# ISU-PAAL/DeepDFA

Measured on NVIDIA H100. Metric: CFG graphs/sec (train step), higher is better.
Workload: dtype f32 (GRU GEMMs: bf16x3 split operands, f32 accumulate)

## Files before the change

deepdfa_b200/csrc/gru_tc_bwd.cu:

```cuda
#include <cuda_fp16.h>

#include <atomic>

#include "tc_common.cuh"

namespace ddfa {
namespace tc2b {
using namespace tcc;

constexpr int kThreads = 320, kEpiWarps = 8;

constexpr int kGbWarps = 8;
struct GbRow {
  float4 d, hv, rr, zz, nn, gh;
  float deg;
  int tb, te;
};
__device__ __forceinline__ float4 bf16x4_to_f4(const uint2 &p) {
  return make_float4(__uint_as_float(p.x << 16), __uint_as_float(p.x & 0xffff0000u), __uint_as_float(p.y << 16), __uint_as_float(p.y & 0xffff0000u));
}
__device__ __forceinline__ void gb_load(GbRow &x, const float *__restrict__ dh_out, const float *__restrict__ h,
                                        const uint8_t *__restrict__ h_img_src, const float *__restrict__ gates,
                                        const uint4 *__restrict__ gates_packed, const int32_t *__restrict__ indptr,
                                        const int32_t *__restrict__ indptr_t, size_t plane, int64_t node, int col, bool ok,
// ... 346 lines not shown
    mbar_init(w_full, 1);
    mbar_fence_init();
  }
  __syncthreads();
  if (threadIdx.x == 0) trace_stamp(tron, 0, 0);
  pdl_launch_dependents();

  if (warp == kEpiWarps) {
    const uint64_t pol_saved = l2_policy((hints & 2) ? 1 : 0), pol_dh = l2_policy((hints & 8) ? 1 : 0);
    const uint64_t pol_q = l2_policy((hints & 64) ? 1 : 0);
    if (my_tiles > 0 && elect_one()) {
      mbar_arrive_expect_tx(w_full, kD3WBytes);
      bulk_g2s(sbase, packed3 + (size_t)rh * kD3WBytes, kD3WBytes, w_full);
    }
    __syncwarp();
    pdl_wait();
    int cc = 0;
    for (int k = 0; k < my_tiles; ++k, cc += 4) {
      const int tile = tile_of(k);
      if (elect_one()) {
        const int stage = cc % kD3Stages, use = cc / kD3Stages;
        if (use > 0) mbar_wait_bounded(empty(stage), (use - 1) & 1);
        const int64_t r0 = (int64_t)tile * kTileM + kGtRows * rh;
        const int valid = (int)max((int64_t)0, min((int64_t)kGtRows, (int64_t)N - r0));
        const uint32_t dst = sbase + kD3OffStage + stage * kD3StageBytes;
        const uint32_t bytes = (uint32_t)valid * (kD * 4 + kD * 8) + (HF32 ? (uint32_t)valid * kD * 4 : (uint32_t)kGtRows * kD * 4);
        mbar_arrive_expect_tx(full(stage), bytes);
        if (valid > 0) {
          bulk_g2s_hint(dst + kGtOffD, dh_out + r0 * kD, (uint32_t)valid * kD * 4, full(stage), pol_dh);
          bulk_g2s_hint(dst + kGtOffG, gates_packed + r0 * kD, (uint32_t)valid * kD * 8, full(stage), pol_saved);
        }
        if (HF32) {
          if (valid > 0) bulk_g2s_hint(dst + kGtOffH, h + r0 * kD, (uint32_t)valid * kD * 4, full(stage), pol_saved);
        } else {
          const uint8_t *t0 = h_img_src + (size_t)tile * kImageTileBytes + (size_t)(kGtRows * rh) * 128;
#pragma unroll
          for (int ch = 0; ch < 4; ++ch) bulk_g2s_hint(dst + kGtOffH + ch * (kGtRows * 128), t0 + (size_t)ch * kChunkBytes, kGtRows * 128, full(stage), pol_saved);
        }
      }
      __syncwarp();
      cluster_arrive_release();
      cluster_wait_acquire();
      if (elect_one()) {
        fence_proxy_async_global();
        for (int g = 0; g < 3; ++g) {
          const int m = g < 2 ? g : (role == 0 ? 2 : 3);
          const int c = cc + 1 + g, stage = c % kD3Stages, use = c / kD3Stages;
          if (use > 0) mbar_wait_bounded(empty(stage), (use - 1) & 1);
          mbar_arrive_expect_tx(full(stage), kD3StageBytes);
          bulk_g2s_hint(sbase + kD3OffStage + stage * kD3StageBytes, q_img + (size_t)m * img_stride + (size_t)tile * kImageTileBytes,
                        kD3StageBytes, full(stage), pol_q);
          if (g != 1) trace_stamp(tron, k, g == 0 ? 1 : 2);
        }
      }
      __syncwarp();
    }
  } else {
    pdl_wait();
    const int col = lane * 4;
#define DDFA_POL_TMP l2_policy((hints & 4) ? 2 : 0)
    const int wg = warp >> 2;
    const bool tr = (warp == 0 && lane == 0);
    float4 sum[7];
#pragma unroll
    for (int i = 0; i < 7; ++i) sum[i] = make_float4(0.f, 0.f, 0.f, 0.f);
    static_assert(kGtPre == 2 && kGtRowsPerWarp == 4, "lane slots below assume four rows per warp and two prefetched neighbours per row");
    auto node_of = [&](int tile, int r) { return (int64_t)tile * kTileM + kGtRows * rh + warp + kEpiWarps * r; };
    auto load_scalars = [&](int kk) -> int {
      int v = 0;
      if (kk < my_tiles && lane < 16) {
        const int64_t nd = node_of(tile_of(kk), (lane >> 1) & 3);
        const int32_t *base = lane < 8 ? indptr : indptr_t;
        if (nd < N && base) v = __ldcg(base + nd + (lane & 1));
      }
      return v;
    };
    auto load_ids = [&](int sc) -> int {
      const int r_ = (lane >> 1) & 3, q_ = lane & 1;
      const int tb_ = __shfl_sync(0xffffffffu, sc, 8 + 2 * r_), te_ = __shfl_sync(0xffffffffu, sc, 9 + 2 * r_);
      int v = -1;
      if (lane >= 16 && lane < 24 && tb_ + q_ < te_) v = __ldcg(indices_t + tb_ + q_);
      return v;
    };
    int sc_cur = 0, sc_next = 0, id_cur = -1;
    if constexpr (CSRP) {
      sc_cur = load_scalars(0); sc_next = load_scalars(1);
      id_cur = load_ids(sc_cur);
    }
    int cc = 0;
    for (int k = 0; k < my_tiles; ++k) {
      const int tile = tile_of(k);
      {
        const int stage = cc % kD3Stages, use = cc / kD3Stages;
        ++cc;
        const int64_t node0 = node_of(tile, 0);
        bool ok[kGtRowsPerWarp];
        int tb[kGtRowsPerWarp], te[kGtRowsPerWarp];
        float deg[kGtRowsPerWarp];
        int id[kGtRowsPerWarp][kGtPre];
        if constexpr (CSRP) {
          const int sc_next2 = load_scalars(k + 2);
          const int id_next = load_ids(sc_next);
#pragma unroll
          for (int r = 0; r < kGtRowsPerWarp; ++r) {
            ok[r] = node0 + kEpiWarps * r < N;
            deg[r] = (float)(__shfl_sync(0xffffffffu, sc_cur, 2 * r + 1) - __shfl_sync(0xffffffffu, sc_cur, 2 * r));
            tb[r] = __shfl_sync(0xffffffffu, sc_cur, 8 + 2 * r); te[r] = __shfl_sync(0xffffffffu, sc_cur, 9 + 2 * r);
#pragma unroll
            for (int q = 0; q < kGtPre; ++q) id[r][q] = __shfl_sync(0xffffffffu, id_cur, 16 + 2 * r + q);
          }
          sc_cur = sc_next; sc_next = sc_next2; id_cur = id_next;
        } else {
#pragma unroll
          for (int r = 0; r < kGtRowsPerWarp; ++r) {
            const int64_t nd = node0 + kEpiWarps * r;
            ok[r] = nd < N;
            tb[r] = te[r] = 0;
            deg[r] = 0.f;
            if (ok[r]) {
              deg[r] = (float)(__ldcg(indptr + nd + 1) - __ldcg(indptr + nd));
              if (indptr_t) { tb[r] = __ldcg(indptr_t + nd); te[r] = __ldcg(indptr_t + nd + 1); }
            }
          }
#pragma unroll
          for (int r = 0; r < kGtRowsPerWarp; ++r)
#pragma unroll
            for (int q = 0; q < kGtPre; ++q) id[r][q] = (tb[r] + q < te[r]) ? __ldcg(indices_t + tb[r] + q) : -1;
        }
        float4 gv[kGtRowsPerWarp][kGtPre];
#pragma unroll
        for (int r = 0; r < kGtRowsPerWarp; ++r)
#pragma unroll
          for (int q = 0; q < kGtPre; ++q) gv[r][q] = id[r][q] >= 0 ? ldg_cg_f4(ds_in + (size_t)id[r][q] * kD + col) : make_float4(0.f, 0.f, 0.f, 0.f);
        mbar_wait_bounded(full(stage), use & 1);
        const uint8_t *st = smem + kD3OffStage + stage * kD3StageBytes;
#pragma unroll
        for (int r = 0; r < kGtRowsPerWarp; ++r) {
          const int row = warp + kEpiWarps * r;
          float4 d = make_float4(0.f, 0.f, 0.f, 0.f), hv = d, rr = d, zz = d, nn = d, gh = d;
          if (ok[r]) {
            d = *reinterpret_cast<const float4 *>(st + kGtOffD + row * (kD * 4) + col * 4);
            const uint4 g0 = *reinterpret_cast<const uint4 *>(st + kGtOffG + row * (kD * 8) + col * 8);
            const uint4 g1 = *reinterpret_cast<const uint4 *>(st + kGtOffG + row * (kD * 8) + col * 8 + 16);
            unpack_gates(make_uint2(g0.x, g0.y), rr.x, zz.x, nn.x, gh.x);
            unpack_gates(make_uint2(g0.z, g0.w), rr.y, zz.y, nn.y, gh.y);
            unpack_gates(make_uint2(g1.x, g1.y), rr.z, zz.z, nn.z, gh.z);
            unpack_gates(make_uint2(g1.z, g1.w), rr.w, zz.w, nn.w, gh.w);
            if (HF32) {
              hv = *reinterpret_cast<const float4 *>(st + kGtOffH + row * (kD * 4) + col * 4);
            } else {
              const uint32_t off = (uint32_t)((col >> 6) * (kGtRows * 128) + row * 128 + (((((col & 63) >> 3) ^ (row & 7)) & 7) << 4) + (col & 7) * 2);
              const uint2 hh = *reinterpret_cast<const uint2 *>(st + kGtOffH + off);
              const uint2 hl = *reinterpret_cast<const uint2 *>(st + kGtOffH + 2 * (kGtRows * 128) + off);
              const float4 a = bf16x4_to_f4(hh), b = bf16x4_to_f4(hl);
              hv = make_float4(a.x + b.x, a.y + b.y, a.z + b.z, a.w + b.w);
            }
#pragma unroll
            for (int q = 0; q < kGtPre; ++q) f4_add(d, gv[r][q]);
            for (int j = tb[r] + kGtPre; j < te[r]; ++j) f4_add(d, ldg_cg_f4(ds_in + (size_t)__ldcg(indices_t + j) * kD + col));
          }
          float4 qr = make_float4(0.f, 0.f, 0.f, 0.f), qz = qr, qn = qr, qnr = qr;
          const int64_t node = node0 + kEpiWarps * r;
          if (ok[r]) {
            st_f4_hint(dh + (size_t)node * kD + col, make_float4(d.x * zz.x, d.y * zz.y, d.z * zz.z, d.w * zz.w), DDFA_POL_TMP);
#define BWDQ2(f)                                         \
  {                                                      \
    const float dz_ = d.f * (hv.f - nn.f);               \
    const float dn_ = d.f * (1.f - zz.f);                \
    qn.f = dn_ * (1.f - nn.f * nn.f);                    \
    qz.f = dz_ * zz.f * (1.f - zz.f);                    \
    qr.f = qn.f * gh.f * rr.f * (1.f - rr.f);            \
    qnr.f = qn.f * rr.f;                                 \
  }
            BWDQ2(x) BWDQ2(y) BWDQ2(z) BWDQ2(w)
#undef BWDQ2
            f4_add(sum[0], qr); f4_add(sum[1], qz); f4_add(sum[2], qn); f4_add(sum[3], qnr);
            f4_fma(sum[4], deg[r], qr); f4_fma(sum[5], deg[r], qz); f4_fma(sum[6], deg[r], qn);
          }
          const size_t o_hi = image_offset(node, col, 0), o_lo = image_offset(node, col, 1);
          uint2 ph, pl;
          split4(qr, ph, pl);  *reinterpret_cast<uint2 *>(q_img + 0 * img_stride + o_hi) = ph; *reinterpret_cast<uint2 *>(q_img + 0 * img_stride + o_lo) = pl;
          split4(qz, ph, pl);  *reinterpret_cast<uint2 *>(q_img + 1 * img_stride + o_hi) = ph; *reinterpret_cast<uint2 *>(q_img + 1 * img_stride + o_lo) = pl;
          split4(qn, ph, pl);  *reinterpret_cast<uint2 *>(q_img + 2 * img_stride + o_hi) = ph; *reinterpret_cast<uint2 *>(q_img + 2 * img_stride + o_lo) = pl;
          split4(qnr, ph, pl); *reinterpret_cast<uint2 *>(q_img + 3 * img_stride + o_hi) = ph; *reinterpret_cast<uint2 *>(q_img + 3 * img_stride + o_lo) = pl;
        }
        __syncwarp();
        if (lane == 0) mbar_arrive(empty(stage));
      }
      if (k > 0 && (warp & 3) == 0) {
        bulk_wait_read_all();
        __syncwarp();
        if (lane == 0) mbar_arrive_n(empty(kD3OutStage), kEpiWarps / 2);
      }
      fence_proxy_async_global();
      cluster_arrive_release();
      cluster_wait_acquire();
      if (tr) trace_stamp(tron, k, 11);
      if ((warp & 3) == 0 && role == 1) fence_proxy_async_global();
      if (k == 0) mbar_wait_bounded(w_full, 0);
      float acc[32];
      int pending = -1;
      if (tr) { trace_stamp(tron, k, 7); trace_stamp(tron, k, 3); }
      for (int g = 0; g < 3; ++g, ++cc) {
        const int stage = cc % kD3Stages, use = cc / kD3Stages;
        mbar_wait_bounded(full(stage), use & 1);
        if (tr && g != 1) trace_stamp(tron, k, g == 0 ? 4 : 5);
        wgmma_fence();
        const uint32_t a0 = sbase + kD3OffStage + stage * kD3StageBytes + wg * 8192;
        const uint32_t w0 = sbase + g * 4 * kD3WChunkBytes;
#pragma unroll
        for (int kb = 0; kb < 2; ++kb) {
#pragma unroll
          for (int k4 = 0; k4 < 4; ++k4) {
            const uint64_t a_hi = gmma_desc(a0 + kb * kChunkBytes + k4 * 32), a_lo = gmma_desc(a0 + (2 + kb) * kChunkBytes + k4 * 32);
            const uint64_t b_hi = gmma_desc(w0 + kb * kD3WChunkBytes + k4 * 32), b_lo = gmma_desc(w0 + (2 + kb) * kD3WChunkBytes + k4 * 32);
            wgmma_n64<0, 0>(acc, a_hi, b_hi, (g == 0 && kb == 0 && k4 == 0) ? 0u : 1u);
            wgmma_n64<0, 0>(acc, a_hi, b_lo, 1u);
            wgmma_n64<0, 0>(acc, a_lo, b_hi, 1u);
          }
        }
        wgmma_commit();
        wgmma_wait<1>();
        __syncwarp();
        if (pending >= 0 && lane == 0) mbar_arrive(empty(pending));
        pending = stage;
      }
      wgmma_wait<0>();
      wgmma_fence_regs(acc);
      if (tr) { trace_stamp(tron, k, 6); trace_stamp(tron, k, 8); trace_stamp(tron, k, 9); }
      const uint32_t st_base = sbase + kD3OffStage + kD3OutStage * kD3StageBytes;
      if (wg == 0) asm volatile("bar.sync 2, 128;" ::: "memory");
      else asm volatile("bar.sync 3, 128;" ::: "memory");
      uint32_t tid;
      asm volatile("mov.u32 %0, %%tid.x;" : "=r"(tid));
#pragma unroll
      for (int hh = 0; hh < 2; ++hh) {
        const uint32_t rowp = staged_row(st_base, wg, (tid >> 5 & 3) * 16 + (tid >> 2 & 7) + 8 * hh) + 8 * (tid & 3);
#pragma unroll
        for (int j = 0; j < 8; ++j)
          asm volatile("st.shared.v2.f32 [%0], {%1, %2};" ::"r"(rowp + 32 * j), "f"(acc[4 * j + 2 * hh]), "f"(acc[4 * j + 2 * hh + 1]) : "memory");
      }
      fence_proxy_async_shared();
      if (wg == 0) asm volatile("bar.sync 2, 128;" ::: "memory");
      else asm volatile("bar.sync 3, 128;" ::: "memory");
      if ((warp & 3) == 0 && elect_one()) {
        const uint64_t pol_tmp = DDFA_POL_TMP;
        const int64_t node0 = (int64_t)tile * kTileM + wg * 64;
        float *out = (role == 0 ? ds : dh) + node0 * kD + half * 64;
        const int rows = (int)min((int64_t)64, (int64_t)N - node0);
        for (int r = 0; r < rows; ++r) {
          if (role == 0) bulk_s2g_hint(out + (int64_t)r * kD, staged_row(st_base, wg, r), 64 * 4, pol_tmp);
          else bulk_s2g_add_f32_hint(out + (int64_t)r * kD, staged_row(st_base, wg, r), 64 * 4, pol_tmp);
        }
        bulk_commit();
      }
      __syncwarp();
      if (tr) trace_stamp(tron, k, 10);
    }
#undef DDFA_POL_TMP
    bulk_wait_all();
    asm volatile("bar.sync 1, %0;" ::"n"(32 * kEpiWarps) : "memory");
    float *red = reinterpret_cast<float *>(smem + kD3OffStage);
#pragma unroll
    for (int i = 0; i < 7; ++i) *reinterpret_cast<float4 *>(&red[(warp * 7 + i) * kD + col]) = sum[i];
  }
  __syncthreads();
  const float *red = reinterpret_cast<const float *>(smem + kD3OffStage);
  for (int i = threadIdx.x; i < 7 * kD; i += kD3Threads) {
    float v_ = 0.f;
#pragma unroll
    for (int w = 0; w < kEpiWarps; ++w) v_ += red[(w * 7) * kD + i];
    if (bias_slots) { bias_slots[(size_t)blockIdx.x * 7 * kD + i] = v_; continue; }
    const int which = i >> 7, c_ = i & 127;
    if (which == 0) { atomicAdd(db_ih + c_, v_); atomicAdd(db_hh + c_, v_); }
    else if (which == 1) { atomicAdd(db_ih + kD + c_, v_); atomicAdd(db_hh + kD + c_, v_); }
    else if (which == 2) atomicAdd(db_ih + 2 * kD + c_, v_);
    else if (which == 3) atomicAdd(db_hh + 2 * kD + c_, v_);
    else atomicAdd(db_fold + (which - 4) * kD + c_, v_);
  }
}

constexpr int kWgSlotBytes = kImageTileBytes;
constexpr int kWgSlots = 3;
constexpr int kWgOffBar = kWgSlots * kWgSlotBytes;
constexpr int kWgSmemAlloc = kWgOffBar + 2 * kWgSlots * 8 + 1024;
constexpr int kWgThreads = 32 * kEpiWarps + 32;
constexpr size_t kWgPartialFloats = (size_t)3 * kD * kD;
constexpr int kWgMaxSteps = 16;
struct WgBatch {
  const uint8_t *s_img[kWgMaxSteps];
  const uint8_t *h_img[kWgMaxSteps];
  int32_t steps;
};
__global__ void __launch_bounds__(kWgThreads, 1) wgrad_kernel(const uint8_t *__restrict__ q_img, size_t img_stride, size_t step_stride,
                                                              const __grid_constant__ WgBatch batch,
                                                              int32_t N, float *__restrict__ partial, int first, int hints) {
  extern __shared__ uint8_t smem_raw[];
  uint8_t *smem = reinterpret_cast<uint8_t *>((reinterpret_cast<uintptr_t>(smem_raw) + 1023) & ~(uintptr_t)1023);
  const uint32_t sbase = smem_u32(smem);
  const uint32_t bar0 = sbase + kWgOffBar;
  auto full = [&](int i) { return bar0 + 8u * i; };
  auto empty = [&](int i) { return bar0 + 8u * (kWgSlots + i); };

  const int warp = threadIdx.x >> 5, lane = threadIdx.x & 31;
  const int role = blockIdx.y / 3, g = blockIdx.y % 3;
  const int qm = g < 2 ? g : (role == 0 ? 2 : 3);
  const int num_tiles = (N + kTileM - 1) / kTileM;
  const int all_tiles = num_tiles * batch.steps;
  const int my_tiles = (all_tiles > (int)blockIdx.x) ? (all_tiles - 1 - (int)blockIdx.x) / (int)gridDim.x + 1 : 0;

  if (threadIdx.x == 0) {
    for (int i = 0; i < kWgSlots; ++i) { mbar_init(full(i), 1); mbar_init(empty(i), kEpiWarps); }
    mbar_fence_init();
  }
  __syncthreads();
  const int tron = (g_trace_on == 2) && blockIdx.y == 0;
  if (threadIdx.x == 0) trace_stamp(tron, 0, 0);

  if (warp == kEpiWarps) {
    if (elect_one()) {
      const uint64_t pol_wg = l2_policy((hints & 32) ? 1 : 0);
      for (int i = 0; i < my_tiles; ++i) {
        const int idx = (int)blockIdx.x + i * (int)gridDim.x;
        const int t = idx / num_tiles, tile = idx - t * num_tiles;
        for (int w = 0; w < 2; ++w) {
// ... 283 lines not shown
```

deepdfa_b200/csrc/tc_common.cuh:

```cuda
#pragma once
#include <cuda_bf16.h>

#include "common.cuh"

namespace ddfa {
namespace tcc {

constexpr int kD = 128;
constexpr int kTileM = 128;
constexpr int kChunkBytes = 128 * 128;
constexpr int kImageTileBytes = 4 * kChunkBytes;

__host__ __device__ __forceinline__ size_t image_bytes(int64_t n) { return (size_t)((n + kTileM - 1) / kTileM) * kImageTileBytes; }

__device__ __forceinline__ uint32_t smem_u32(const void *p) { return (uint32_t)__cvta_generic_to_shared(p); }

__device__ __forceinline__ void mbar_init(uint32_t bar, uint32_t count) {
  asm volatile("mbarrier.init.shared::cta.b64 [%0], %1;" ::"r"(bar), "r"(count));
}
__device__ __forceinline__ void mbar_fence_init() { asm volatile("fence.mbarrier_init.release.cluster;" ::: "memory"); }
__device__ __forceinline__ void mbar_arrive(uint32_t bar) {
  asm volatile("mbarrier.arrive.shared::cta.b64 _, [%0];" ::"r"(bar) : "memory");
}
__device__ __forceinline__ void mbar_arrive_expect_tx(uint32_t bar, uint32_t bytes) {
// ... 80 lines not shown

__device__ __forceinline__ void mbar_wait_bounded(uint32_t bar, uint32_t parity) {
  for (uint32_t it = 0; it < (1u << 24); ++it) {
    uint32_t done;
    asm volatile(
        "{\n"
        ".reg .pred p;\n"
        "mbarrier.try_wait.parity.shared::cta.b64 p, [%1], %2;\n"
        "selp.u32 %0, 1, 0, p;\n"
        "}\n"
        : "=r"(done)
        : "r"(bar), "r"(parity)
        : "memory");
    if (done) return;
  }
  __trap();
}


__host__ __device__ __forceinline__ uint32_t sw128_offset(int row, int k) {
  return (uint32_t)((row >> 3) * 1024 + (row & 7) * 128 + ((((k >> 3) ^ (row & 7)) & 7) << 4) + (k & 7) * 2);
}
__host__ __device__ __forceinline__ size_t image_offset(int64_t node, int col, int v) {
  return (size_t)(node / kTileM) * kImageTileBytes + (size_t)((v * 2 + (col >> 6)) * kChunkBytes) +
         sw128_offset((int)(node % kTileM), col & 63);
}

__device__ __forceinline__ void split_bf16(float x, __nv_bfloat16 &hi, __nv_bfloat16 &lo) {
  hi = __float2bfloat16_rn(x);
  lo = __float2bfloat16_rn(x - __bfloat162float(hi));
}
__device__ __forceinline__ uint32_t bf16x2_bits(float lo_half, float hi_half) {
  const __nv_bfloat162 v = __floats2bfloat162_rn(lo_half, hi_half);
  return *reinterpret_cast<const uint32_t *>(&v);
}
__device__ __forceinline__ void split4(const float4 &x, uint2 &ph, uint2 &pl) {
  ph.x = bf16x2_bits(x.x, x.y);
  ph.y = bf16x2_bits(x.z, x.w);
  pl.x = bf16x2_bits(x.x - __uint_as_float(ph.x << 16), x.y - __uint_as_float(ph.x & 0xffff0000u));
  pl.y = bf16x2_bits(x.z - __uint_as_float(ph.y << 16), x.w - __uint_as_float(ph.y & 0xffff0000u));
}
__device__ __forceinline__ void split8(const float (&x)[8], uint4 &ph, uint4 &pl) {
  uint2 h0, l0, h1, l1;
  split4(make_float4(x[0], x[1], x[2], x[3]), h0, l0);
  split4(make_float4(x[4], x[5], x[6], x[7]), h1, l1);
  ph = make_uint4(h0.x, h0.y, h1.x, h1.y);
  pl = make_uint4(l0.x, l0.y, l1.x, l1.y);
}

__device__ __forceinline__ uint2 pack_gates(float r, float z, float n, float ghn) {
  const uint32_t rq = __float_as_uint(fmaf(r, 16383.f, 8388608.f)) & 0x3fffu, zq = __float_as_uint(fmaf(z, 16383.f, 8388608.f)) & 0x3fffu;
  const uint32_t nq = __float_as_uint(fmaf(n, 32767.f, 12582912.f)) & 0xffffu;
  const uint32_t b = __float_as_uint(ghn);
  const int core = (int)(((b + 0x100u) << 1) >> 10) - (112 << 14);
  uint32_t g = core < (1 << 14) ? 0u : (uint32_t)min(core, (31 << 14) - 1);
  g |= (b >> 12) & 0x80000u;
  return make_uint2(rq | (zq << 14) | (g << 28), nq | ((g >> 4) << 16));
}
__device__ __forceinline__ void unpack_gates(const uint2 &p, float &r, float &z, float &n, float &ghn) {
  r = (float)(p.x & 0x3fffu) * (1.f / 16383.f);
  z = (float)((p.x >> 14) & 0x3fffu) * (1.f / 16383.f);
  n = (__uint_as_float(((p.y & 0xffffu) ^ 0x4b008000u)) - 8421376.f) * (1.f / 32767.f);
  const uint32_t g = ((p.y >> 16) << 4) | (p.x >> 28);
  const uint32_t e = (g >> 14) & 31u;
  ghn = e == 0u ? 0.f : __uint_as_float(((g >> 19) << 31) | ((e + 112u) << 23) | ((g & 0x3fffu) << 9));
}

__device__ __forceinline__ float ex2_ftz(float x) {
  float y;
  asm("ex2.approx.ftz.f32 %0, %1;" : "=f"(y) : "f"(x));
  return y;
}
__device__ __forceinline__ float rcp_ftz(float x) {
  float y;
  asm("rcp.approx.ftz.f32 %0, %1;" : "=f"(y) : "f"(x));
  return y;
}
__device__ __forceinline__ float fast_sigmoid(float x) { return rcp_ftz(1.f + ex2_ftz(-1.4426950408889634f * x)); }
__device__ __forceinline__ float fast_tanh(float x) {
  const float e = ex2_ftz(2.885390081777927f * x);
  return fmaf(-2.f, rcp_ftz(e + 1.f), 1.f);
}

constexpr int kTraceCtas = 132, kTraceTiles = 12, kTraceEvents = 12;
constexpr size_t kTraceWords = (size_t)kTraceCtas * kTraceTiles * kTraceEvents;
static __device__ long long g_trace[kTraceWords];
static __device__ int g_trace_on = 0;
__device__ __forceinline__ void trace_stamp(int on, int tile_i, int ev) {
  if (on && blockIdx.x < kTraceCtas && tile_i < kTraceTiles)
    g_trace[((size_t)blockIdx.x * kTraceTiles + tile_i) * kTraceEvents + ev] = clock64();
}

}
}
```

deepdfa_b200/csrc/gru_tc_fwd3.cu:

```cuda
#include <cuda_fp16.h>
#include <stdlib.h>

#include "tc_common.cuh"

namespace ddfa {
namespace tc3 {
using namespace tcc;

constexpr int kSlices = 4;
constexpr int kSliceCols = kD / kSlices;
constexpr int kRowsPerPart = 3 * kSliceCols;
constexpr int kWChunkBytes = kRowsPerPart * 128;
constexpr int kSliceWBytes = 8 * kWChunkBytes;
constexpr int kStageBytes = kImageTileBytes;
constexpr int kOffStage = kSliceWBytes;
constexpr int kOffBias = kOffStage + 2 * kStageBytes;
constexpr int kBiasSlice = 7 * kSliceCols;
constexpr int kOffBar = kOffBias + kBiasSlice * 4;
constexpr int kSmemAlloc = kOffBar + 5 * 8;
constexpr int kConsumerWarps = 8;
constexpr int kThreads = 32 * kConsumerWarps + 32;
constexpr size_t kPackedWBytes = (size_t)kSlices * kSliceWBytes;
constexpr size_t kPackedBytes = kPackedWBytes + (size_t)kSlices * kBiasSlice * 4;
static_assert(kSmemAlloc <= 232448, "shared memory budget");

__global__ void pack_kernel(const float *__restrict__ w_fold, const float *__restrict__ w_hh, const float *__restrict__ b_fold,
                            const float *__restrict__ b_ih, const float *__restrict__ b_hh, uint8_t *__restrict__ packed) {
  const int idx = blockIdx.x * blockDim.x + threadIdx.x;
  if (idx >= kSlices * 2 * kRowsPerPart * 16) return;
  const int u = idx % 16, n = (idx / 16) % kRowsPerPart, p = (idx / (16 * kRowsPerPart)) % 2, slice = idx / (32 * kRowsPerPart);
  const int kb = u >> 3, k0 = u * 8;
  const float *W = (p == 0 ? w_fold : w_hh) + (size_t)((n / kSliceCols) * kD + slice * kSliceCols + n % kSliceCols) * kD;
  float x[8];
#pragma unroll
  for (int i = 0; i < 8; ++i) x[i] = W[k0 + i];
  uint4 ph, pl;
  split8(x, ph, pl);
  uint8_t *base = packed + (size_t)slice * kSliceWBytes + sw128_offset(n, (u & 7) * 8);
  *reinterpret_cast<uint4 *>(base + ((p * 2 + 0) * 2 + kb) * kWChunkBytes) = ph;
  *reinterpret_cast<uint4 *>(base + ((p * 2 + 1) * 2 + kb) * kWChunkBytes) = pl;
  if (p == 0 && u == 0 && n < kSliceCols) {
    const int t = slice * kSliceCols + n;
    float *bias = reinterpret_cast<float *>(packed + kPackedWBytes) + slice * kBiasSlice;
    bias[0 * kSliceCols + n] = b_ih[2 * kD + t];
    bias[1 * kSliceCols + n] = b_ih[t] + b_hh[t];
    bias[2 * kSliceCols + n] = b_ih[kD + t] + b_hh[kD + t];
    bias[3 * kSliceCols + n] = b_hh[2 * kD + t];
    bias[4 * kSliceCols + n] = b_fold[2 * kD + t];
    bias[5 * kSliceCols + n] = b_fold[t];
    bias[6 * kSliceCols + n] = b_fold[kD + t];
  }
}

template <bool HIMG, int GATES>
__global__ void __launch_bounds__(kThreads, 1) gru_fwd3_kernel(const uint8_t *__restrict__ s_img, const uint8_t *__restrict__ h_img,
                                                               const float *__restrict__ h, const int32_t *__restrict__ indptr,
                                                               const uint8_t *__restrict__ packed, int32_t N,
                                                               float *__restrict__ h_out, uint8_t *__restrict__ h_out_img,
                                                               float *__restrict__ gates, uint2 *__restrict__ gates_packed, int hints) {
  extern __shared__ __align__(1024) uint8_t smem[];
  const uint32_t sbase = smem_u32(smem);
  if ((sbase & 1023u) != 0) __trap();
  const uint32_t bar0 = sbase + kOffBar;
  auto full = [&](int i) { return bar0 + 8u * i; };
  auto empty = [&](int i) { return bar0 + 8u * (2 + i); };
  const uint32_t w_full = bar0 + 32u;

  const int warp = threadIdx.x >> 5, lane = threadIdx.x & 31;
  const int slice = blockIdx.x % kSlices;
  const int group = blockIdx.x / kSlices, num_groups = gridDim.x / kSlices;
  const int num_tiles = (N + kTileM - 1) / kTileM;
  const int my_tiles = (num_tiles > group) ? (num_tiles - 1 - group) / num_groups + 1 : 0;

  if (threadIdx.x == 0) {
    for (int i = 0; i < 2; ++i) { mbar_init(full(i), 1); mbar_init(empty(i), kConsumerWarps); }
    mbar_init(w_full, 1);
    mbar_fence_init();
  }
  __syncthreads();
  const int tron = g_trace_on;
  if (threadIdx.x == 0) trace_stamp(tron, 0, 0);
  pdl_launch_dependents();

  if (warp == kConsumerWarps) {
    if (my_tiles > 0 && elect_one()) {
      mbar_arrive_expect_tx(w_full, kSliceWBytes);
      bulk_g2s(sbase, packed + (size_t)slice * kSliceWBytes, kSliceWBytes, w_full);
      pdl_wait();
      for (int k = 0; k < my_tiles; ++k) {
        const size_t toff = (size_t)(group + k * num_groups) * kImageTileBytes;
        for (int p = 0; p < 2; ++p) {
          if (k > 0) mbar_wait_bounded(empty(p), (k - 1) & 1);
          mbar_arrive_expect_tx(full(p), kStageBytes);
          bulk_g2s(sbase + kOffStage + p * kStageBytes, (p == 0 ? s_img : h_img) + toff, kStageBytes, full(p));
          trace_stamp(tron, k, 1 + p);
        }
      }
    }
    return;
  }

  float *sbias = reinterpret_cast<float *>(smem + kOffBias);
  for (int i = threadIdx.x; i < kBiasSlice; i += 32 * kConsumerWarps)
    sbias[i] = __ldcg(reinterpret_cast<const float *>(packed + kPackedWBytes) + slice * kBiasSlice + i);
  asm volatile("bar.sync 1, %0;" ::"n"(32 * kConsumerWarps) : "memory");
  pdl_wait();
  if (my_tiles == 0) return;
  const int wg = warp >> 2;
  const int row0 = wg * 64 + (warp & 3) * 16 + (lane >> 2);
  const int c4 = 2 * (lane & 3);
  const size_t plane = (size_t)N * kD;
  const uint64_t pol_gates = l2_policy((hints & 1) ? 1 : 0);
  const uint64_t pol_next = l2_policy((hints & 16) ? 2 : 0);
  mbar_wait_bounded(w_full, 0);
  const bool tr = (warp == 0 && lane == 0);

  for (int k = 0; k < my_tiles; ++k) {
    const int tile = group + k * num_groups;
    float acc_s[48], acc_h[48];
    if (tr) { trace_stamp(tron, k, 7); trace_stamp(tron, k, 3); }
    mbar_wait_bounded(full(0), k & 1);
    if (tr) trace_stamp(tron, k, 4);
    wgmma_fence();
#pragma unroll
    for (int p = 0; p < 2; ++p) {
      if (p == 1) {
        mbar_wait_bounded(full(1), k & 1);
        if (tr) trace_stamp(tron, k, 5);
      }
      const uint32_t a0 = sbase + kOffStage + p * kStageBytes + wg * 8192;
      const uint32_t w0 = sbase + p * 4 * kWChunkBytes;
#pragma unroll
      for (int kb = 0; kb < 2; ++kb) {
#pragma unroll
        for (int k4 = 0; k4 < 4; ++k4) {
          const uint64_t a_hi = gmma_desc(a0 + kb * kChunkBytes + k4 * 32), a_lo = gmma_desc(a0 + (2 + kb) * kChunkBytes + k4 * 32);
          const uint64_t b_hi = gmma_desc(w0 + kb * kWChunkBytes + k4 * 32), b_lo = gmma_desc(w0 + (2 + kb) * kWChunkBytes + k4 * 32);
          const uint32_t acc = (kb == 0 && k4 == 0) ? 0u : 1u;
          if (p == 0) {
            wgmma_n96<0, 0>(acc_s, a_hi, b_hi, acc);
            wgmma_n96<0, 0>(acc_s, a_hi, b_lo, 1u);
            wgmma_n96<0, 0>(acc_s, a_lo, b_hi, 1u);
          } else {
            wgmma_n96<0, 0>(acc_h, a_hi, b_hi, acc);
            wgmma_n96<0, 0>(acc_h, a_hi, b_lo, 1u);
            wgmma_n96<0, 0>(acc_h, a_lo, b_hi, 1u);
          }
        }
      }
      wgmma_commit();
    }
    float deg[2], hp[2][8];
#pragma unroll
    for (int hh = 0; hh < 2; ++hh) {
      const int64_t node = (int64_t)tile * kTileM + row0 + 8 * hh;
      const bool valid = node < N;
      deg[hh] = valid ? (float)(__ldcg(indptr + node + 1) - __ldcg(indptr + node)) : 0.f;
#pragma unroll
      for (int j = 0; j < 4; ++j) {
        const int gcol = slice * kSliceCols + 8 * j + c4;
        if constexpr (HIMG) {
          const uint32_t whi = __ldcg(reinterpret_cast<const uint32_t *>(h_img + image_offset(node, gcol, 0)));
          const uint32_t wlo = __ldcg(reinterpret_cast<const uint32_t *>(h_img + image_offset(node, gcol, 1)));
          hp[hh][2 * j] = __uint_as_float(whi << 16) + __uint_as_float(wlo << 16);
          hp[hh][2 * j + 1] = __uint_as_float(whi & 0xffff0000u) + __uint_as_float(wlo & 0xffff0000u);
        } else {
          const float2 v = valid ? __ldcg(reinterpret_cast<const float2 *>(h + node * kD + gcol)) : make_float2(0.f, 0.f);
          hp[hh][2 * j] = v.x;
          hp[hh][2 * j + 1] = v.y;
        }
      }
    }
    wgmma_wait<0>();
    wgmma_fence_regs(acc_s);
    wgmma_fence_regs(acc_h);
    if (tr) { trace_stamp(tron, k, 6); trace_stamp(tron, k, 8); }
    __syncwarp();
    if (lane == 0) { mbar_arrive(empty(0)); mbar_arrive(empty(1)); }
    if (tr) trace_stamp(tron, k, 9);

#pragma unroll
    for (int hh = 0; hh < 2; ++hh) {
      const int64_t node = (int64_t)tile * kTileM + row0 + 8 * hh;
      const bool valid = node < N;
#pragma unroll
      for (int j = 0; j < 4; ++j) {
        const int c = 8 * j + c4, gcol = slice * kSliceCols + c;
        float hn[2], rr[2], zz[2], nn[2], gg[2];
#pragma unroll
        for (int e = 0; e < 2; ++e) {
          const int i = 2 * hh + e;
          const float dg = deg[hh];
          const float gin = acc_s[4 * (8 + j) + i] + fmaf(dg, sbias[4 * kSliceCols + c + e], sbias[c + e]);
          const float r = fast_sigmoid(acc_s[4 * j + i] + acc_h[4 * j + i] + fmaf(dg, sbias[5 * kSliceCols + c + e], sbias[kSliceCols + c + e]));
          const float z = fast_sigmoid(acc_s[4 * (4 + j) + i] + acc_h[4 * (4 + j) + i] +
                                       fmaf(dg, sbias[6 * kSliceCols + c + e], sbias[2 * kSliceCols + c + e]));
          const float ghn = acc_h[4 * (8 + j) + i] + sbias[3 * kSliceCols + c + e];
          const float n = fast_tanh(fmaf(r, ghn, gin));
          hn[e] = valid ? fmaf(z, hp[hh][2 * j + e] - n, n) : 0.f;
          rr[e] = r; zz[e] = z; nn[e] = n; gg[e] = ghn;
        }
        const size_t off = (size_t)node * kD + gcol;
        if (valid && h_out != nullptr) st_f2_hint(h_out + off, make_float2(hn[0], hn[1]), pol_next);
        if constexpr (GATES == 2) {
          if (valid) {
            const uint2 g0 = pack_gates(rr[0], zz[0], nn[0], gg[0]), g1 = pack_gates(rr[1], zz[1], nn[1], gg[1]);
            st_u4_hint(gates_packed + off, make_uint4(g0.x, g0.y, g1.x, g1.y), pol_gates);
          }
        }
        if constexpr (GATES == 1) {
          if (valid) {
            st_f2_hint(gates + off, make_float2(rr[0], rr[1]), pol_gates);
            st_f2_hint(gates + plane + off, make_float2(zz[0], zz[1]), pol_gates);
            st_f2_hint(gates + 2 * plane + off, make_float2(nn[0], nn[1]), pol_gates);
            st_f2_hint(gates + 3 * plane + off, make_float2(gg[0], gg[1]), pol_gates);
          }
        }
        if (h_out_img != nullptr) {
          const uint32_t hw = bf16x2_bits(hn[0], hn[1]);
          const uint32_t lw = bf16x2_bits(hn[0] - __uint_as_float(hw << 16), hn[1] - __uint_as_float(hw & 0xffff0000u));
          st_u32_hint(h_out_img + image_offset(node, gcol, 0), hw, pol_next);
          st_u32_hint(h_out_img + image_offset(node, gcol, 1), lw, pol_next);
        }
      }
    }
    if (tr) trace_stamp(tron, k, 10);
  }
}

}

size_t gru_tc3_packed_bytes() { return tc3::kPackedBytes; }

int gru_tc3_prepare(const float *w_fold, const float *b_fold, const float *b_ih, const float *w_hh, const float *b_hh, void *packed,
                    cudaStream_t stream) {
  const int total = tc3::kSlices * 2 * tc3::kRowsPerPart * 16;
  tc3::pack_kernel<<<(total + 127) / 128, 128, 0, stream>>>(w_fold, w_hh, b_fold, b_ih, b_hh, static_cast<uint8_t *>(packed));
  DDFA_CHECK_LAUNCH("tc3::pack_kernel");
  chain_break();
  return DDFA_OK;
}

int gru_tc3_step_fwd(const void *s_img, const void *h_img, const float *h, const int32_t *indptr, int32_t N, float *h_out,
                     void *h_out_img, float *save_gates, void *save_gates_packed, const void *packed, cudaStream_t stream) {
  const int tiles = (N + tcc::kTileM - 1) / tcc::kTileM;
  int groups = kNumSMs / tc3::kSlices;
  if (groups > tiles) groups = tiles;
  if (save_gates && save_gates_packed) {
    set_error("tcgen05 engine (fwd): both gate formats requested");
    return DDFA_ERR_INVALID_ARG;
  }
  if ((h == nullptr && save_gates) ) {
    set_error("tcgen05 engine (fwd): fp32 gate planes go with the fp32 h operand (legacy form)");
    return DDFA_ERR_INVALID_ARG;
  }
  if (tiles == 0) return DDFA_OK;
#define DDFA_FWD3_LAUNCH(HIMG, GATES)                                                                                                     \
  do {                                                                                                                                   \
    DDFA_CUDA(cudaFuncSetAttribute(tc3::gru_fwd3_kernel<HIMG, GATES>, cudaFuncAttributeMaxDynamicSharedMemorySize, tc3::kSmemAlloc));     \
    DDFA_CUDA(launch_chain(2, tc3::gru_fwd3_kernel<HIMG, GATES>, dim3(groups * tc3::kSlices), dim3(tc3::kThreads), tc3::kSmemAlloc,        \
                           stream, static_cast<const uint8_t *>(s_img), static_cast<const uint8_t *>(h_img), h, indptr,                   \
                           static_cast<const uint8_t *>(packed), N, h_out, static_cast<uint8_t *>(h_out_img), save_gates,                \
                           static_cast<uint2 *>(save_gates_packed), l2_hints()));                                                        \
  } while (0)
  if (h) {
    if (save_gates) DDFA_FWD3_LAUNCH(false, 1);
    else if (save_gates_packed) DDFA_FWD3_LAUNCH(false, 2);
    else DDFA_FWD3_LAUNCH(false, 0);
  } else {
    if (save_gates_packed) DDFA_FWD3_LAUNCH(true, 2);
    else DDFA_FWD3_LAUNCH(true, 0);
  }
#undef DDFA_FWD3_LAUNCH
  DDFA_CHECK_LAUNCH("tc3::gru_fwd3_kernel");
  return DDFA_OK;
}

namespace tc3 {
__global__ void __launch_bounds__(256) to_image_kernel(const float *__restrict__ x, int32_t N, uint8_t *__restrict__ image) {
  const int64_t t = blockIdx.x * (int64_t)blockDim.x + threadIdx.x;
  const int64_t rows = ((int64_t)N + kTileM - 1) / kTileM * kTileM;
  if (t >= rows * 16) return;
  const int64_t node = t >> 4;
  const int col = (int)(t & 15) * 8;
  float v[8] = {0.f, 0.f, 0.f, 0.f, 0.f, 0.f, 0.f, 0.f};
  if (node < N) {
    const float4 a = ldg_nc_f4(x + node * kD + col), b = ldg_nc_f4(x + node * kD + col + 4);
    v[0] = a.x; v[1] = a.y; v[2] = a.z; v[3] = a.w; v[4] = b.x; v[5] = b.y; v[6] = b.z; v[7] = b.w;
  }
  uint4 ph, pl;
  split8(v, ph, pl);
  *reinterpret_cast<uint4 *>(image + image_offset(node, col, 0)) = ph;
  *reinterpret_cast<uint4 *>(image + image_offset(node, col, 1)) = pl;
}
}

size_t act_image_bytes(int64_t n) { return tcc::image_bytes(n); }

int act_to_image(const float *x, int32_t N, void *image, cudaStream_t stream) {
  const int64_t rows = ((int64_t)N + tcc::kTileM - 1) / tcc::kTileM * tcc::kTileM;
  const int64_t total = rows * 16;
  if (total == 0) return DDFA_OK;
  tc3::to_image_kernel<<<(unsigned)((total + 255) / 256), 256, 0, stream>>>(x, N, static_cast<uint8_t *>(image));
  DDFA_CHECK_LAUNCH("to_image_kernel");
  return DDFA_OK;
}

size_t gru_tc2_workspace_bytes() { return gru_tc3_packed_bytes(); }

// ... 31 lines not shown
```

Measured before the change: 120,500.

## Prefetch next tile's neighbour ds rows during the store phase of the backward gather

For the CSR-prefetch, bf16-image path, the first two transposed-neighbour rows of ds_in for the next tile are now loaded into registers (gvn) right after the previous tile's accumulator staging, instead of at the start of the tile. This is meant to hide gather latency behind the bulk store and the cluster barrier. The stage counter is also recomputed per tile, and extra trace stamps are added, with the trace event count raised. The cost is extra live float4 registers across the loop, which risks register pressure.

Measured after the change: 120,500 (median of 6 runs). Within noise of the previous version (-0.0%).

```diff
diff --git a/deepdfa_b200/csrc/gru_tc_bwd.cu b/deepdfa_b200/csrc/gru_tc_bwd.cu
--- a/deepdfa_b200/csrc/gru_tc_bwd.cu
+++ b/deepdfa_b200/csrc/gru_tc_bwd.cu
@@ -452,14 +452,26 @@
       if (lane >= 16 && lane < 24 && tb_ + q_ < te_) v = __ldcg(indices_t + tb_ + q_);
       return v;
     };
+    constexpr bool kRowsAhead = CSRP && !HF32;
+    float4 gvn[kGtRowsPerWarp][kGtPre];
+    auto request_rows = [&](int ids) {
+#pragma unroll
+      for (int r = 0; r < kGtRowsPerWarp; ++r)
+#pragma unroll
+        for (int q = 0; q < kGtPre; ++q) {
+          const int i_ = __shfl_sync(0xffffffffu, ids, 16 + 2 * r + q);
+          gvn[r][q] = i_ >= 0 ? ldg_cg_f4(ds_in + (size_t)i_ * kD + col) : make_float4(0.f, 0.f, 0.f, 0.f);
+        }
+    };
     int sc_cur = 0, sc_next = 0, id_cur = -1;
     if constexpr (CSRP) {
       sc_cur = load_scalars(0); sc_next = load_scalars(1);
       id_cur = load_ids(sc_cur);
-    }
-    int cc = 0;
+      if constexpr (kRowsAhead) request_rows(id_cur);
+    }
     for (int k = 0; k < my_tiles; ++k) {
       const int tile = tile_of(k);
+      int cc = 4 * k;
       {
         const int stage = cc % kD3Stages, use = cc / kD3Stages;
         ++cc;
@@ -467,7 +479,7 @@
         bool ok[kGtRowsPerWarp];
         int tb[kGtRowsPerWarp], te[kGtRowsPerWarp];
         float deg[kGtRowsPerWarp];
-        int id[kGtRowsPerWarp][kGtPre];
+        float4 gv[kGtRowsPerWarp][kGtPre];
         if constexpr (CSRP) {
           const int sc_next2 = load_scalars(k + 2);
           const int id_next = load_ids(sc_next);
@@ -477,10 +489,18 @@
             deg[r] = (float)(__shfl_sync(0xffffffffu, sc_cur, 2 * r + 1) - __shfl_sync(0xffffffffu, sc_cur, 2 * r));
             tb[r] = __shfl_sync(0xffffffffu, sc_cur, 8 + 2 * r); te[r] = __shfl_sync(0xffffffffu, sc_cur, 9 + 2 * r);
 #pragma unroll
-            for (int q = 0; q < kGtPre; ++q) id[r][q] = __shfl_sync(0xffffffffu, id_cur, 16 + 2 * r + q);
+            for (int q = 0; q < kGtPre; ++q) {
+              if constexpr (kRowsAhead) {
+                gv[r][q] = gvn[r][q];
+              } else {
+                const int i_ = __shfl_sync(0xffffffffu, id_cur, 16 + 2 * r + q);
+                gv[r][q] = i_ >= 0 ? ldg_cg_f4(ds_in + (size_t)i_ * kD + col) : make_float4(0.f, 0.f, 0.f, 0.f);
+              }
+            }
           }
           sc_cur = sc_next; sc_next = sc_next2; id_cur = id_next;
         } else {
+          int id[kGtRowsPerWarp][kGtPre];
 #pragma unroll
           for (int r = 0; r < kGtRowsPerWarp; ++r) {
             const int64_t nd = node0 + kEpiWarps * r;
@@ -496,13 +516,13 @@
           for (int r = 0; r < kGtRowsPerWarp; ++r)
 #pragma unroll
             for (int q = 0; q < kGtPre; ++q) id[r][q] = (tb[r] + q < te[r]) ? __ldcg(indices_t + tb[r] + q) : -1;
-        }
-        float4 gv[kGtRowsPerWarp][kGtPre];
-#pragma unroll
-        for (int r = 0; r < kGtRowsPerWarp; ++r)
-#pragma unroll
-          for (int q = 0; q < kGtPre; ++q) gv[r][q] = id[r][q] >= 0 ? ldg_cg_f4(ds_in + (size_t)id[r][q] * kD + col) : make_float4(0.f, 0.f, 0.f, 0.f);
+#pragma unroll
+          for (int r = 0; r < kGtRowsPerWarp; ++r)
+#pragma unroll
+            for (int q = 0; q < kGtPre; ++q) gv[r][q] = id[r][q] >= 0 ? ldg_cg_f4(ds_in + (size_t)id[r][q] * kD + col) : make_float4(0.f, 0.f, 0.f, 0.f);
+        }
         mbar_wait_bounded(full(stage), use & 1);
+        if (tr) trace_stamp(tron, k, 13);
         const uint8_t *st = smem + kD3OffStage + stage * kD3StageBytes;
 #pragma unroll
         for (int r = 0; r < kGtRowsPerWarp; ++r) {
@@ -527,6 +547,10 @@
             }
 #pragma unroll
             for (int q = 0; q < kGtPre; ++q) f4_add(d, gv[r][q]);
+            if (r == 0 && tr) {
+              asm volatile("" ::"f"(d.x), "f"(d.y), "f"(d.z), "f"(d.w));
+              trace_stamp(tron, k, 12);
+            }
             for (int j = tb[r] + kGtPre; j < te[r]; ++j) f4_add(d, ldg_cg_f4(ds_in + (size_t)__ldcg(indices_t + j) * kD + col));
           }
           float4 qr = make_float4(0.f, 0.f, 0.f, 0.f), qz = qr, qn = qr, qnr = qr;
@@ -555,6 +579,7 @@
           split4(qnr, ph, pl); *reinterpret_cast<uint2 *>(q_img + 3 * img_stride + o_hi) = ph; *reinterpret_cast<uint2 *>(q_img + 3 * img_stride + o_lo) = pl;
         }
         __syncwarp();
+        if (tr) trace_stamp(tron, k, 14);
         if (lane == 0) mbar_arrive(empty(stage));
       }
       if (k > 0 && (warp & 3) == 0) {
@@ -563,6 +588,7 @@
         if (lane == 0) mbar_arrive_n(empty(kD3OutStage), kEpiWarps / 2);
       }
       fence_proxy_async_global();
+      if (tr) trace_stamp(tron, k, 15);
       cluster_arrive_release();
       cluster_wait_acquire();
       if (tr) trace_stamp(tron, k, 11);
@@ -611,6 +637,7 @@
           asm volatile("st.shared.v2.f32 [%0], {%1, %2};" ::"r"(rowp + 32 * j), "f"(acc[4 * j + 2 * hh]), "f"(acc[4 * j + 2 * hh + 1]) : "memory");
       }
       fence_proxy_async_shared();
+      if constexpr (kRowsAhead) request_rows(id_cur);
       if (wg == 0) asm volatile("bar.sync 2, 128;" ::: "memory");
       else asm volatile("bar.sync 3, 128;" ::: "memory");
       if ((warp & 3) == 0 && elect_one()) {
diff --git a/deepdfa_b200/csrc/tc_common.cuh b/deepdfa_b200/csrc/tc_common.cuh
--- a/deepdfa_b200/csrc/tc_common.cuh
+++ b/deepdfa_b200/csrc/tc_common.cuh
@@ -186,7 +186,7 @@
   return fmaf(-2.f, rcp_ftz(e + 1.f), 1.f);
 }
 
-constexpr int kTraceCtas = 132, kTraceTiles = 12, kTraceEvents = 12;
+constexpr int kTraceCtas = 132, kTraceTiles = 12, kTraceEvents = 16;
 constexpr size_t kTraceWords = (size_t)kTraceCtas * kTraceTiles * kTraceEvents;
 static __device__ long long g_trace[kTraceWords];
 static __device__ int g_trace_on = 0;
```

## Split tile staging per warpgroup and interleave WGMMA issue with ping-pong barriers

Applied to the files above, without the earlier changes.

Splits each staged activation tile into per-warpgroup halves with their own full/empty barriers, so each warpgroup waits only on its own 64-row half and frees it on its own. Adds named-barrier turn-taking so the two warpgroups take turns issuing WGMMA, letting one warpgroup's epilogue overlap the other's tensor-core work. Also reads the previous hidden state from the already-staged shared-memory image instead of reloading it from global memory. The cost is four copies per slot instead of one bulk copy, and extra barrier handshakes that could add stalls or deadlock if the turn logic is off.

New measurement: 120,100 before, 123,300 after, median of 6. 2.7% higher.

```diff
diff --git a/deepdfa_b200/csrc/gru_tc_fwd3.cu b/deepdfa_b200/csrc/gru_tc_fwd3.cu
--- a/deepdfa_b200/csrc/gru_tc_fwd3.cu
+++ b/deepdfa_b200/csrc/gru_tc_fwd3.cu
@@ -12,14 +12,16 @@
 constexpr int kRowsPerPart = 3 * kSliceCols;
 constexpr int kWChunkBytes = kRowsPerPart * 128;
 constexpr int kSliceWBytes = 8 * kWChunkBytes;
-constexpr int kStageBytes = kImageTileBytes;
-constexpr int kOffStage = kSliceWBytes;
-constexpr int kOffBias = kOffStage + 2 * kStageBytes;
+constexpr int kPieceBytes = kChunkBytes / 2;
+constexpr int kSlotBytes = 4 * kPieceBytes;
+constexpr int kOffSlot = kSliceWBytes;
+constexpr int kOffBias = kOffSlot + 4 * kSlotBytes;
 constexpr int kBiasSlice = 7 * kSliceCols;
 constexpr int kOffBar = kOffBias + kBiasSlice * 4;
-constexpr int kSmemAlloc = kOffBar + 5 * 8;
+constexpr int kSmemAlloc = kOffBar + 9 * 8;
 constexpr int kConsumerWarps = 8;
 constexpr int kThreads = 32 * kConsumerWarps + 32;
+constexpr int kBarTurn0 = 2, kBarTurn1 = 3;
 constexpr size_t kPackedWBytes = (size_t)kSlices * kSliceWBytes;
 constexpr size_t kPackedBytes = kPackedWBytes + (size_t)kSlices * kBiasSlice * 4;
 static_assert(kSmemAlloc <= 232448, "shared memory budget");
@@ -63,8 +65,9 @@
   if ((sbase & 1023u) != 0) __trap();
   const uint32_t bar0 = sbase + kOffBar;
   auto full = [&](int i) { return bar0 + 8u * i; };
-  auto empty = [&](int i) { return bar0 + 8u * (2 + i); };
-  const uint32_t w_full = bar0 + 32u;
+  auto empty = [&](int i) { return bar0 + 8u * (4 + i); };
+  auto slot = [&](int i) { return sbase + kOffSlot + i * kSlotBytes; };
+  const uint32_t w_full = bar0 + 64u;
 
   const int warp = threadIdx.x >> 5, lane = threadIdx.x & 31;
   const int slice = blockIdx.x % kSlices;
@@ -73,7 +76,7 @@
   const int my_tiles = (num_tiles > group) ? (num_tiles - 1 - group) / num_groups + 1 : 0;
 
   if (threadIdx.x == 0) {
-    for (int i = 0; i < 2; ++i) { mbar_init(full(i), 1); mbar_init(empty(i), kConsumerWarps); }
+    for (int i = 0; i < 4; ++i) { mbar_init(full(i), 1); mbar_init(empty(i), kConsumerWarps / 2); }
     mbar_init(w_full, 1);
     mbar_fence_init();
   }
@@ -89,11 +92,15 @@
       pdl_wait();
       for (int k = 0; k < my_tiles; ++k) {
         const size_t toff = (size_t)(group + k * num_groups) * kImageTileBytes;
-        for (int p = 0; p < 2; ++p) {
-          if (k > 0) mbar_wait_bounded(empty(p), (k - 1) & 1);
-          mbar_arrive_expect_tx(full(p), kStageBytes);
-          bulk_g2s(sbase + kOffStage + p * kStageBytes, (p == 0 ? s_img : h_img) + toff, kStageBytes, full(p));
-          trace_stamp(tron, k, 1 + p);
+        for (int w = 0; w < 2; ++w) {
+          for (int p = 0; p < 2; ++p) {
+            const int i = 2 * w + p;
+            if (k > 0) mbar_wait_bounded(empty(i), (k - 1) & 1);
+            mbar_arrive_expect_tx(full(i), kSlotBytes);
+            const uint8_t *src = (p == 0 ? s_img : h_img) + toff + w * kPieceBytes;
+            for (int c = 0; c < 4; ++c) bulk_g2s(slot(i) + c * kPieceBytes, src + c * kChunkBytes, kPieceBytes, full(i));
+            trace_stamp(tron, 2 * k + w, 1 + p);
+          }
         }
       }
     }
@@ -113,28 +120,40 @@
   const uint64_t pol_gates = l2_policy((hints & 1) ? 1 : 0);
   const uint64_t pol_next = l2_policy((hints & 16) ? 2 : 0);
   mbar_wait_bounded(w_full, 0);
-  const bool tr = (warp == 0 && lane == 0);
+  const bool tr = ((warp & 3) == 0 && lane == 0);
+  auto wait_turn = [&]() {
+    if (wg == 0) asm volatile("bar.sync %0, %1;" ::"n"(kBarTurn0), "n"(32 * kConsumerWarps) : "memory");
+    else asm volatile("bar.sync %0, %1;" ::"n"(kBarTurn1), "n"(32 * kConsumerWarps) : "memory");
+  };
+  auto pass_turn = [&]() {
+    if (wg == 0) asm volatile("bar.arrive %0, %1;" ::"n"(kBarTurn1), "n"(32 * kConsumerWarps) : "memory");
+    else asm volatile("bar.arrive %0, %1;" ::"n"(kBarTurn0), "n"(32 * kConsumerWarps) : "memory");
+  };
+  const int rl = row0 - wg * 64;
 
   for (int k = 0; k < my_tiles; ++k) {
     const int tile = group + k * num_groups;
+    const int ts = 2 * k + wg;
     float acc_s[48], acc_h[48];
-    if (tr) { trace_stamp(tron, k, 7); trace_stamp(tron, k, 3); }
-    mbar_wait_bounded(full(0), k & 1);
-    if (tr) trace_stamp(tron, k, 4);
+    if (tr) trace_stamp(tron, ts, 7);
+    mbar_wait_bounded(full(2 * wg), k & 1);
+    if (tr) trace_stamp(tron, ts, 4);
+    if (wg == 1 || k > 0) wait_turn();
+    if (tr) trace_stamp(tron, ts, 3);
     wgmma_fence();
 #pragma unroll
     for (int p = 0; p < 2; ++p) {
       if (p == 1) {
-        mbar_wait_bounded(full(1), k & 1);
-        if (tr) trace_stamp(tron, k, 5);
-      }
-      const uint32_t a0 = sbase + kOffStage + p * kStageBytes + wg * 8192;
+        mbar_wait_bounded(full(2 * wg + 1), k & 1);
+        if (tr) trace_stamp(tron, ts, 5);
+      }
+      const uint32_t a0 = slot(2 * wg + p);
       const uint32_t w0 = sbase + p * 4 * kWChunkBytes;
 #pragma unroll
       for (int kb = 0; kb < 2; ++kb) {
 #pragma unroll
         for (int k4 = 0; k4 < 4; ++k4) {
-          const uint64_t a_hi = gmma_desc(a0 + kb * kChunkBytes + k4 * 32), a_lo = gmma_desc(a0 + (2 + kb) * kChunkBytes + k4 * 32);
+          const uint64_t a_hi = gmma_desc(a0 + kb * kPieceBytes + k4 * 32), a_lo = gmma_desc(a0 + (2 + kb) * kPieceBytes + k4 * 32);
           const uint64_t b_hi = gmma_desc(w0 + kb * kWChunkBytes + k4 * 32), b_lo = gmma_desc(w0 + (2 + kb) * kWChunkBytes + k4 * 32);
           const uint32_t acc = (kb == 0 && k4 == 0) ? 0u : 1u;
           if (p == 0) {
@@ -150,6 +169,8 @@
       }
       wgmma_commit();
     }
+    if (wg == 0 || k + 1 < my_tiles) pass_turn();
+    if (tr) trace_stamp(tron, ts, 11);
     float deg[2], hp[2][8];
 #pragma unroll
     for (int hh = 0; hh < 2; ++hh) {
@@ -160,8 +181,9 @@
       for (int j = 0; j < 4; ++j) {
         const int gcol = slice * kSliceCols + 8 * j + c4;
         if constexpr (HIMG) {
-          const uint32_t whi = __ldcg(reinterpret_cast<const uint32_t *>(h_img + image_offset(node, gcol, 0)));
-          const uint32_t wlo = __ldcg(reinterpret_cast<const uint32_t *>(h_img + image_offset(node, gcol, 1)));
+          const uint8_t *hs = smem + kOffSlot + (2 * wg + 1) * kSlotBytes + (gcol >> 6) * kPieceBytes + sw128_offset(rl + 8 * hh, gcol & 63);
+          const uint32_t whi = *reinterpret_cast<const uint32_t *>(hs);
+          const uint32_t wlo = *reinterpret_cast<const uint32_t *>(hs + 2 * kPieceBytes);
           hp[hh][2 * j] = __uint_as_float(whi << 16) + __uint_as_float(wlo << 16);
           hp[hh][2 * j + 1] = __uint_as_float(whi & 0xffff0000u) + __uint_as_float(wlo & 0xffff0000u);
         } else {
@@ -174,10 +196,10 @@
     wgmma_wait<0>();
     wgmma_fence_regs(acc_s);
     wgmma_fence_regs(acc_h);
-    if (tr) { trace_stamp(tron, k, 6); trace_stamp(tron, k, 8); }
+    if (tr) { trace_stamp(tron, ts, 6); trace_stamp(tron, ts, 8); }
     __syncwarp();
-    if (lane == 0) { mbar_arrive(empty(0)); mbar_arrive(empty(1)); }
-    if (tr) trace_stamp(tron, k, 9);
+    if (lane == 0) { mbar_arrive(empty(2 * wg)); mbar_arrive(empty(2 * wg + 1)); }
+    if (tr) trace_stamp(tron, ts, 9);
 
 #pragma unroll
     for (int hh = 0; hh < 2; ++hh) {
@@ -224,7 +246,7 @@
         }
       }
     }
-    if (tr) trace_stamp(tron, k, 10);
+    if (tr) trace_stamp(tron, ts, 10);
   }
 }
 
```
